# Sytronik/thesia

Measured on AMD Instinct MI355X. Metric: STFT frames/sec (whole step: STFT->dB->min/max->u16 image->level-0 RGBA raster), n_fft=2048, higher is better.
Workload: dtype f32

## Files before the change

__graft_entry__.py:

```python
from __future__ import annotations

import os
import shutil
import subprocess
import sys

ROOT = os.path.dirname(os.path.abspath(__file__))
CSRC = os.path.join(ROOT, "thesia_amd", "csrc")
LIB = os.path.join(ROOT, "thesia_amd", "libthesia_amd.so")
OBJDIR = os.path.join(ROOT, "build", "obj")
SOURCES = ["kernels_stft_w2048.hip", "kernels_stft_w4096.hip", "kernels_stft_w1024.hip", "kernels_stft.hip", "api.hip", "track_manager.hip", "track_manager_multi.hip", "kernels_stft_long.hip",
           "kernels_mel.hip", "kernels_image.hip", "kernels_waveform.hip", "kernels_loudness.hip", "kernels_dynamics.hip", "kernels_spectrum.hip", "kernels_meter.hip", "kernels_export.hip", "kernels_resample.hip", "host_math.cpp", "reader_plan.cpp", "batch_plan.cpp", "tile_cache.cpp"]
EXTRA_FLAGS = {"kernels_image.hip": ["-ffp-contract=off"], "kernels_waveform.hip": ["-ffp-contract=off"],
               "kernels_loudness.hip": ["-ffp-contract=off"],
               "kernels_dynamics.hip": ["-ffp-contract=off"],
               "kernels_spectrum.hip": ["-ffp-contract=off"],
               "kernels_meter.hip": ["-ffp-contract=off"],
               "kernels_export.hip": ["-ffp-contract=off"],
               "kernels_resample.hip": ["-ffp-contract=off", "-fno-slp-vectorize"],
               "kernels_stft.hip": ["-fno-slp-vectorize"] + os.environ.get("TH_STFT_EXTRA_FLAGS", "").split(),
               "kernels_stft_w1024.hip": ["-fno-slp-vectorize"] + os.environ.get("TH_STFT_EXTRA_FLAGS", "").split(),
               "kernels_stft_w2048.hip": ["-fno-slp-vectorize"] + os.environ.get("TH_STFT_EXTRA_FLAGS", "").split(),
               "kernels_stft_w4096.hip": ["-fno-slp-vectorize"] + os.environ.get("TH_STFT_EXTRA_FLAGS", "").split(),
               "kernels_stft_long.hip": ["-fno-slp-vectorize"]}
HEADERS = ["batch_plan.h", "common.h", "context.h", "export_core.h", "host_math.h", "kernels.h", "mel_fuse.h", "plan_error.h", "reader_plan.h", "resample_block.h", "resample_core.h", "stft_core.h", "stft_plan.h", "stft_pk.h", "stft_wave.h", "stft_wave_multi.h", "stft_block.h", "tile_cache.h", "track_manager_internal.h",
           "../../include/thesia_amd.h", "../../include/thesia_amd_testing.h"]


def _hipcc() -> str:
    for cand in (shutil.which("hipcc"), "/opt/rocm/bin/hipcc"):
        if cand and os.path.exists(cand):
            return cand
    raise RuntimeError("hipcc not found")


def _stale(target: str, deps) -> bool:
    if not os.path.exists(target):
        return True
    t = os.path.getmtime(target)
    return any(os.path.getmtime(d) > t for d in deps if os.path.exists(d))


def build(force: bool = False) -> None:
    import fcntl
    os.makedirs(OBJDIR, exist_ok=True)
    with open(os.path.join(OBJDIR, ".lock"), "w") as lock:
        fcntl.flock(lock, fcntl.LOCK_EX)
        try:
            _build_locked(force)
# ... 84 lines not shown
```

include/thesia_amd_testing.h:

```cpp
#ifndef THESIA_AMD_TESTING_H
#define THESIA_AMD_TESTING_H

#include "thesia_amd.h"

TH_API int th_plan_set_kernel(th_plan *plan, int which);

TH_API int th_build_ab_variants(void);

TH_API int th_plan_mel_moments_info(const th_plan *plan, uint32_t *n_groups, uint32_t *taps, double *max_dev, double *max_amp);

TH_API int th_plan_time_kernel(th_plan *plan, int enable);
TH_API int th_plan_kernel_ms_history(th_plan *plan, float *out_ms, size_t capacity, size_t *n_out);
TH_API int th_plan_last_kernel_ms(th_plan *plan, float *ms);

TH_API int th_tm_put_img(th_tm *tm, size_t id, uint32_t ch, const uint16_t *img, size_t height, size_t width);

#endif
```

thesia_amd/_ffi.py:

```python
from __future__ import annotations

import ctypes as C
import importlib.util
import os
import sys

_HERE = os.path.dirname(os.path.abspath(__file__))
LIB_PATH = os.environ.get("THESIA_AMD_LIB") or os.path.join(_HERE, "libthesia_amd.so")

if not os.path.exists(LIB_PATH):
    raise ImportError(
        f"{LIB_PATH} not found: build the HIP extension first "
        "(python -c 'import __graft_entry__ as g; g.build()').  thesia_amd has no CPU fallback."
    )



def _preload_hip_runtime() -> None:
    if "torch" in sys.modules or os.environ.get("THESIA_AMD_SYSTEM_HIP") == "1":
        return
    try:
        spec = importlib.util.find_spec("torch")
    except Exception:
        spec = None
# ... 207 lines not shown
    "th_host_alloc": [vp, C.c_size_t, C.POINTER(C.c_void_p)],
    "th_host_free": [vp, C.c_void_p],
    "th_minmax_reduce_dev": [vp, C.c_void_p, C.c_size_t, C.c_void_p],
    "th_global_db_range_dev": [vp, C.c_void_p, C.c_float, C.c_void_p],
    "th_minmax_reduce_range_dev": [vp, vp, C.c_size_t, C.c_float, vp, vp],
    "th_spec_to_img_batch_dev_ranged": [vp, C.POINTER(ImgDesc), C.c_size_t, C.c_void_p, C.c_uint32],
    "th_plan_time_kernel": [vp, C.c_int],
    "th_plan_last_kernel_ms": [vp, C.POINTER(C.c_float)],
    "th_plan_kernel_ms_history": [vp, c_f32p, C.c_size_t, c_szp],
    "th_channel_stats_dev": [vp, C.POINTER(StatsDesc), C.c_size_t, c_f32p, c_f32p],
    "th_audio_stats_dev": [vp, C.POINTER(AudioDesc), C.c_size_t, C.POINTER(AudioStats)],
    "th_k_weighting": [C.c_uint32, C.POINTER(C.c_double), C.POINTER(C.c_double)],
    "th_loudness_n_blocks": [C.c_size_t, C.c_uint32, c_szp],
    "th_gated_loudness": [C.POINTER(C.c_double), C.c_size_t, C.POINTER(C.c_double)],
    "th_tm_get_audio_stats": [vp, C.c_size_t, C.POINTER(AudioStats)],
    "th_tmg_get_audio_stats": [vp, C.c_size_t, C.POINTER(AudioStats)],
    "th_waveform_pyramid_bins": [C.c_uint64, C.c_uint32],
    "th_waveform_pyramid_offset": [C.c_uint64, C.c_uint32],
    "th_waveform_pyramid_dev": [vp, C.POINTER(PyramidDesc), C.c_size_t],
    "th_tm_tile_cache": [vp, C.POINTER(vp)],
    "th_tm_set_lod_source": [vp, C.c_int],
    "th_tm_mip_level": [vp, C.c_size_t, C.c_uint32, C.c_uint32, C.c_uint32, c_u16p, C.c_size_t, c_szp, c_szp],
    "th_tm_put_img": [vp, C.c_size_t, C.c_uint32, c_u16p, C.c_size_t, C.c_size_t],
    "th_tm_lod_footprint": [vp, c_szp, c_szp, c_szp],
    "th_tm_get_audio_render_metadata": [vp, C.c_size_t, C.c_uint32, C.c_double, C.c_int, C.POINTER(RenderMetadata)],
    "th_tmg_create": [C.POINTER(C.c_int), C.c_size_t, C.POINTER(vp)],
    "th_tmg_destroy": [vp],
    "th_tmg_n_devices": [vp, c_szp],
    "th_tmg_track_device": [vp, C.c_size_t, C.POINTER(C.c_uint32)],
    "th_tmg_set_colormap": [vp, c_u8p, C.c_size_t],
    "th_tmg_set_setting": [vp, C.c_double, C.c_uint32, C.c_uint32, C.c_int],
    "th_tmg_set_dB_range": [vp, C.c_float],
    "th_tmg_add_tracks": [vp, C.c_size_t, c_szp, C.POINTER(C.c_uint32), C.POINTER(C.c_uint32), C.POINTER(c_f32p),
                          c_szp],
    "th_tmg_remove_track": [vp, C.c_size_t],
    "th_tmg_apply_track_list_changes": [vp, c_szp, C.c_size_t, c_szp, C.POINTER(C.c_uint32)],
    "th_tmg_get_db_state": [vp, c_f32p, c_f32p, C.POINTER(C.c_uint32)],
    "th_tmg_spec_shape": [vp, C.c_size_t, C.c_uint32, c_szp, c_szp],
    "th_tmg_img_shape": [vp, C.c_size_t, C.c_uint32, c_szp, c_szp],
    "th_tmg_copy_spec": [vp, C.c_size_t, C.c_uint32, c_f32p, C.c_size_t],
    "th_tmg_copy_img": [vp, C.c_size_t, C.c_uint32, c_u16p, C.c_size_t],
    "th_tmg_revisions": [vp, C.POINTER(C.c_uint64), C.POINTER(C.c_uint64)],
    "th_tmg_get_spectrogram_tile": [vp, C.c_size_t, C.c_uint32, C.c_uint32, C.c_uint32, C.c_uint32, C.c_uint32,
                                    c_u8p, C.c_size_t, c_szp],
    "th_tmg_get_spectrogram_tiles": [vp, C.c_void_p, C.c_size_t, C.c_void_p, C.c_size_t, c_szp, c_szp],
    "th_tmg_get_waveform_tile": [vp, C.c_size_t, C.c_uint32, C.c_uint32, C.c_uint32, c_u8p, C.c_size_t, c_szp],
# ... 77 lines not shown
```

thesia_amd/csrc/api.hip:

```cpp
#include <hip/hip_runtime.h>

#include <cmath>
#include <cstdio>
#include <cstring>
#include <memory>
#include <mutex>
#include <vector>

#include "common.h"
#include "context.h"
#include "export_core.h"
#include "host_math.h"
#include "kernels.h"
#include "mel_fuse.h"
#include "resample_core.h"
#include "track_manager_internal.h"
#if !defined(TH_MEL_BAND_TAPS_2048)
#define TH_MEL_BAND_TAPS_2048 64u
#define TH_MEL_BAND_TAPS_1024 80u
#endif
#if !defined(TH_MEL_BAND_SPREAD)
#define TH_MEL_BAND_SPREAD 1
#endif

// ... 334 lines not shown
}
TH_API int th_timer_start(th_ctx *c) {
    TH_TRY
    TH_REQUIRE(c, "ctx is NULL");
    TH_HIP(hipSetDevice(c->device));
    TH_HIP(hipEventRecord(c->ev0, c->stream));
    return TH_OK;
    TH_CATCH
}
TH_API int th_timer_stop_ms(th_ctx *c, float *ms) {
    TH_TRY
    TH_CHECK(refuse_while_capturing("reading a timer"));
    TH_REQUIRE(c && ms, "NULL argument");
    TH_HIP(hipSetDevice(c->device));
    TH_HIP(hipEventRecord(c->ev1, c->stream));
    TH_HIP(hipEventSynchronize(c->ev1));
    TH_HIP(hipEventElapsedTime(ms, c->ev0, c->ev1));
    return TH_OK;
    TH_CATCH
}

namespace th {

int DeviceTable::ensure(size_t bytes) {
    if (bytes <= cap) return TH_OK;
    TH_CHECK(refuse_while_capturing("allocating a scratch buffer or a descriptor table"));
    if (dptr) {
        TH_HIP(hipFree(dptr));
        dptr = nullptr;
        cap = 0;
    }
    size_t want = bytes < 4096 ? 4096 : bytes + bytes / 2;
    TH_HIP(hipMalloc(&dptr, want));
    cap = want;
    last.clear();
    return TH_OK;
}

int DeviceTable::upload(hipStream_t s, const void *src, size_t bytes) {
    if (bytes == last.size() && bytes && std::memcmp(last.data(), src, bytes) == 0) return TH_OK;
    TH_CHECK(refuse_while_capturing("uploading a descriptor table (a first call, or one with other descriptors)"));
    TH_HIP(hipStreamSynchronize(s));
    int rc = ensure(bytes);
    if (rc != TH_OK) return rc;
    if (bytes) TH_HIP(hipMemcpy(dptr, src, bytes, hipMemcpyHostToDevice));
    last.assign(static_cast<const unsigned char *>(src), static_cast<const unsigned char *>(src) + bytes);
    return TH_OK;
}

void DeviceTable::release() {
    if (dptr) (void)hipFree(dptr);
    dptr = nullptr;
    cap = 0;
    last.clear();
}

}

static void resolve_route(th_plan &p) {
    using R = StftRoute;
    const StftGeom &g = p.g;
    const int k = p.kernel_choice, wv = p.wave_waves;
    R r;
    r.block_plan = stft_is_block_plan(g);
    const bool wave = k != SEL_GENERIC && stft_wave_supported(g) && (g.n_mel == 0 || p.d_mel_bt != nullptr);
    r.no_wave_kernel = k >= SEL_WAVE && !wave;
    r.long_plan = k == SEL_BLOCK ? 1 : k == SEL_SUBWAVE ? 2
                : (g.n_mel != 0 && g.log2_nc == 13 && p.d_mel_mom != nullptr && k != SEL_MEL_TWO_KERNELS) ? 1
                : stft_subwave_default(g) ? 2 : 1;
    bool fused = false, mom_small = false, bsum_fits = false;
    if (g.n_mel != 0 && wave && k != SEL_MEL_AMP && k != SEL_MEL_MFMA) {
        bsum_fits = k != SEL_MEL_PIECES && p.d_mel_bsum != nullptr && stft_wave_mel_fits(g, wv, p.mel_bsum_words, true);
        const bool pieces_fit = p.d_mel_fuse != nullptr && stft_wave_mel_fits(g, wv, p.mel_fuse_words);
        if (g.log2_nc >= 8 && g.log2_nc <= 10 && p.d_mel_mom != nullptr && k != SEL_MEL_TWO_KERNELS && k != SEL_MEL_PIECES)
            mom_small = g.log2_nc == 8 ? p.d_mel_rows == nullptr && stft_wave_multi_applies(g, 2) && stft_wave_multi_mel_fits(g, wv, 0)
                                       : !bsum_fits && !pieces_fit && stft_wave_mel_fits(g, wv, 0, true);
        if (g.log2_nc == 11)
            fused = k != SEL_MEL_TWO_KERNELS && p.d_mel_mom != nullptr && stft_wave_mel_fits(g, wv, 1, true);
        else if (g.log2_nc == 12 || g.log2_nc == 13)
// ... 30 lines not shown
    static const char *const main_name[] = {"stft_generic_kernel", "stft_bluestein_kernel", "stft_wave_kernel", "stft_wave_kernel",
                                            "stft_block_kernel", "stft_subwave_kernel"};
    static const char *const second_name[] = {"", "+mel_rows_kernel", "+mel_band_rows_kernel", "+mel_mfma_kernel"};
    std::snprintf(r.name, sizeof r.name, "%s%s%s", main_name[(int)r.main], fused ? "(fused mel)" : "", second_name[(int)r.mel_second]);
    p.route = r;
}

TH_API int th_plan_create(th_ctx *c, uint32_t sr, size_t win, size_t hop, size_t n_fft, int freq_scale,
                          size_t n_mel, th_plan **out) {
    TH_TRY
    TH_CHECK(refuse_while_capturing("creating a plan"));
    TH_REQUIRE(c && out, "NULL argument");
    *out = nullptr;
    TH_REQUIRE(freq_scale == TH_FREQ_LINEAR || freq_scale == TH_FREQ_MEL, "bad freq_scale %d", freq_scale);
    TH_REQUIRE(win > 1 && hop >= 1 && win <= n_fft, "need 1 < win <= n_fft and hop >= 1 (win=%zu hop=%zu n_fft=%zu)",
               win, hop, n_fft);
    TH_REQUIRE(sr > 0, "sr must be > 0");
    size_t odd_part = n_fft;
    while (odd_part > 1 && odd_part % 2 == 0) odd_part /= 2;
    if (n_fft < 2 || n_fft % 2 != 0 || n_fft > TH_MAX_N_FFT)
        return fail(TH_ERR_UNSUPPORTED, "n_fft=%zu: supported is every even n_fft from 2 to %u", n_fft, (unsigned)TH_MAX_N_FFT);
    TH_HIP(hipSetDevice(c->device));

    std::unique_ptr<th_plan> owner(new th_plan());
    th_plan *p = owner.get();
    p->ctx = c;
    p->sr = sr;
    p->freq_scale = freq_scale;
    StftGeom &g = p->g;
    g = stft_geom(win, hop, n_fft);

    const std::vector<float> w = normalized_hann(win, n_fft);
    const std::vector<cf32> tw = build_twiddles(n_fft);
    {
        const WaveWindowHost ww = build_wave_window(w.data(), win, n_fft, th::stft_wave_phased_mode(g, 0));
        TH_CHECK(p->d_wtab.fill(ww.wtab));
        if (!ww.phased.empty()) TH_CHECK(p->d_wtab_phased.fill(ww.phased));
    }
    TH_CHECK(p->d_window.fill(w));
    {
        const uint32_t zero[4] = {0, 0, 0, 0};
        TH_CHECK(p->d_queue_head.fill(zero, sizeof zero));
    }
    TH_CHECK(p->d_tw.fill(tw));
    if (odd_part > th::STFT_MAX_DIRECT_ODD) {
        const BluesteinTables bt = bluestein_tables(n_fft, th::stft_bluestein_m(g));
        TH_CHECK(p->d_bs_chirp.fill(bt.chirp));
// ... 1039 lines not shown
        dm = static_cast<unsigned char *>(c->loud_mem.dptr);
    }
    b->d_sums = reinterpret_cast<double *>(dm + o_sums);
    double *d_blk = reinterpret_cast<double *>(dm + o_blk), *d_z = reinterpret_cast<double *>(dm + o_z), *d_q = reinterpret_cast<double *>(dm + o_q);
    uint32_t *d_pk = reinterpret_cast<uint32_t *>(dm + o_sums + b->n_ch * 8);
    size_t si = 0;
    for (size_t t = 0, jc = 0; t < n; t++) {
        const size_t q0 = si;
        for (uint32_t k = 0; k < descs[t].n_channels; k++, jc++) {
            LoudJob &j = jobs[jc];
            j.z = d_z + 8 * si;
            j.q = d_q + si;
            j.sumsq = b->d_sums + jc;
            j.peak = d_pk + jc;
            si += j.n_fchunks;
        }
        tjobs[t].q = d_q + q0;
        tjobs[t].out = d_blk + b->blk0[t];
    }
    std::vector<unsigned char> h(o_sums, 0);
    std::memcpy(h.data(), jobs.data(), jobs.size() * sizeof(LoudJob));
    for (size_t r = 0; r < rates.size(); r++) std::memcpy(h.data() + o_rates + r * sizeof(LoudnessRate), rates[r], sizeof(LoudnessRate));
    std::memcpy(h.data() + o_tj, tjobs.data(), tjobs.size() * sizeof(LoudTrackJob));
    TH_HIP(hipMemcpy(dm, h.data(), o_sums, hipMemcpyHostToDevice));
    TH_HIP(hipMemsetAsync(b->d_sums, 0, sums_bytes, c->stream));
    TH_HIP(launch_loudness(reinterpret_cast<const LoudJob *>(dm), (uint32_t)jobs.size(), max_chunks, max_fchunks,
                           reinterpret_cast<const LoudnessRate *>(dm + o_rates), lds_floats, reinterpret_cast<const LoudTrackJob *>(dm + o_tj),
                           (uint32_t)n, max_blocks, c->stream));
    for (size_t t = 0; t < n; t++)
        if (descs[t].block_energy && tjobs[t].n_blocks)
            TH_HIP(hipMemcpyAsync(descs[t].block_energy, tjobs[t].out, tjobs[t].n_blocks * 8, hipMemcpyDeviceToDevice, c->stream));
    return TH_OK;
}

int loudness_collect(LoudnessBatch *b, bool sync_stream) {
    th_ctx *c = b->ctx;
    TH_HIP(hipSetDevice(c->device));
    const size_t sums_bytes = b->n_ch * 8 + (b->n_ch * 4 + 7) / 8 * 8;
    b->h_sums.assign(sums_bytes / 8 + b->n_blocks, 0.0);
    if (sync_stream) {
        TH_HIP(hipMemcpyAsync(b->h_sums.data(), b->d_sums, sums_bytes + b->n_blocks * 8, hipMemcpyDeviceToHost, c->stream));
        TH_HIP(hipStreamSynchronize(c->stream));
    } else {
        TH_HIP(hipMemcpy(b->h_sums.data(), b->d_sums, sums_bytes + b->n_blocks * 8, hipMemcpyDeviceToHost));
    }
    return TH_OK;
}
// ... 39 lines not shown
```

thesia_amd/csrc/context.h:

```cpp
#pragma once
#include <hip/hip_runtime.h>

#include <cstring>
#include <initializer_list>
#include <mutex>
#include <vector>

#include "common.h"
#include "stft_core.h"
#include "stft_plan.h"

namespace th {

template <class T>
struct DeviceBuf {
    T *ptr = nullptr;
    DeviceBuf() = default;
    DeviceBuf(const DeviceBuf &) = delete;
    DeviceBuf &operator=(const DeviceBuf &) = delete;
    DeviceBuf(DeviceBuf &&o) noexcept : ptr(o.ptr) { o.ptr = nullptr; }
    DeviceBuf &operator=(DeviceBuf &&o) noexcept {
        if (this != &o) {
            reset();
            ptr = o.ptr;
            o.ptr = nullptr;
        }
        return *this;
    }
    ~DeviceBuf() { reset(); }
    void reset() {
        if (ptr) (void)hipFree(ptr);
        ptr = nullptr;
    }
    T *get() const { return ptr; }
    operator T *() const { return ptr; }
    hipError_t alloc(size_t bytes) {
        reset();
        return hipMalloc((void **)&ptr, bytes);
    }
    int fill(const void *h, size_t bytes) {
        reset();
        void **d = (void **)&ptr;
        TH_HIP(hipMalloc(d, bytes));
        TH_HIP(hipMemcpy(*d, h, bytes, hipMemcpyHostToDevice));
        return TH_OK;
    }
    template <class V>
    int fill(const std::vector<V> &h) { return fill(h.data(), h.size() * sizeof(V)); }
};

struct DeviceTable {
    void *dptr = nullptr;
    size_t cap = 0;
    std::vector<unsigned char> last;
    int ensure(size_t bytes);
    int upload(hipStream_t s, const void *src, size_t bytes);
    void release();
    DeviceTable() = default;
    DeviceTable(const DeviceTable &) = delete;
    DeviceTable &operator=(const DeviceTable &) = delete;
    ~DeviceTable() { release(); }
};

struct KeyedTables {
    struct Src {
        const void *data;
        size_t bytes;
    };
    DeviceTable tab[3];
    std::vector<unsigned char> key;
    uint32_t n_blocks = 0;
    bool hit(const void *k, size_t bytes) const { return !key.empty() && key.size() == bytes && std::memcmp(key.data(), k, bytes) == 0; }
    int store(hipStream_t s, const void *k, size_t bytes, uint32_t blocks, std::initializer_list<Src> srcs) {
        key.clear();
        size_t i = 0;
        for (const Src &src : srcs) {
            if (src.bytes) TH_CHECK(tab[i].upload(s, src.data, src.bytes));
            i++;
        }
        key.assign(static_cast<const unsigned char *>(k), static_cast<const unsigned char *>(k) + bytes);
        n_blocks = blocks;
        return TH_OK;
    }
    template <class T>
    const T *at(size_t i) const { return static_cast<const T *>(tab[i].dptr); }
};

int refuse_while_capturing(const char *what);

}

struct th_ctx {
    int device = 0;
    uint32_t n_cu = 256;
    hipStream_t stream = nullptr;
    bool own_stream = false;
    hipStream_t capture_stream = nullptr;
    bool capture_swapped = false;
    hipEvent_t ev0 = nullptr, ev1 = nullptr;
    std::recursive_mutex mu;
    th::DeviceTable wave_jobs, wave_start, colormap, tile_out, lod_tabs, lod_tmp, pyr_jobs, pyr_sums, loud_mem;
    th::KeyedTables img, raster, fused;
    ~th_ctx() {
        if (ev0) (void)hipEventDestroy(ev0);
        if (ev1) (void)hipEventDestroy(ev1);
        if (own_stream && stream) (void)hipStreamDestroy(stream);
        if (capture_stream) (void)hipStreamDestroy(capture_stream);
    }
};

struct th_plan {
    th_ctx *ctx = nullptr;
    uint32_t sr = 0;
    int freq_scale = 0;
    int kernel_choice = 0;
    int wave_waves = 0;
    int wave_chunk = 0;
    static constexpr size_t TIMER_SLOTS = 64;
    bool time_kernel = false;
    uint64_t timed_launches = 0;
    std::vector<hipEvent_t> ev_k0, ev_k1;
    th::StftGeom g{};
    th::DeviceBuf<float> d_window;
    th::DeviceBuf<th::cf32> d_tw;
    th::DeviceBuf<double> d_bs_chirp, d_bs_bhat, d_bs_twm, d_bs_tws;
// ... 7 lines not shown
    std::vector<float> h_mel_fb;
    th::DeviceBuf<float> d_mel_bt;
    th::DeviceBuf<uint32_t> d_mel_band, d_mel_slice;
    uint32_t mel_kblocks = 0, mel_ntiles = 0, mel_zero_block = 0, mel_slices = 0;
    th::DeviceBuf<uint32_t> d_mel_rows;
    uint32_t mel_rows_groups = 0;
    th::DeviceTable amp_buf, mel_jobs, mel_tile_start;
    size_t amp_zeroed = 0;
    th::DeviceTable chunk_mm;
    th::DeviceTable gen_scratch;
    th::DeviceTable post_jobs;
    th::DeviceBuf<uint32_t> d_mel_fuse;
    uint32_t mel_fuse_words = 0, mel_fuse_slots = 0, mel_fuse_groups = 0;
    th::DeviceBuf<uint32_t> d_mel_bsum;
    uint32_t mel_bsum_words = 0, mel_bsum_groups = 0, mel_bsum_hdr[16] = {};
    th::DeviceBuf<th::cf32> d_twc;
    uint32_t mel_bsum_reach = 0;
    th::DeviceBuf<uint32_t> d_mel_mom;
    uint32_t mel_mom_groups = 0, mel_mom_taps = 0;
    double mel_mom_max_dev = 0.0, mel_mom_max_amp = 0.0;
    th::DeviceTable jobs, tile_start;
    th::DeviceTable edge_jobs, edge_tile_start;
    th::StftRoute route;
    ~th_plan() {
        for (hipEvent_t e : ev_k0) (void)hipEventDestroy(e);
        for (hipEvent_t e : ev_k1) (void)hipEventDestroy(e);
    }
};

namespace th {
struct LoudnessBatch {
    th_ctx *ctx = nullptr;
    DeviceBuf<unsigned char> d_own;
    double *d_sums = nullptr;
    size_t n_ch = 0, n_blocks = 0;
    std::vector<size_t> ch0, blk0;
    std::vector<uint32_t> srs;
    std::vector<uint64_t> ns;
    std::vector<double> h_blocks;
    std::vector<double> h_sums;
    LoudnessBatch() = default;
    LoudnessBatch(const LoudnessBatch &) = delete;
    LoudnessBatch &operator=(const LoudnessBatch &) = delete;
    ~LoudnessBatch();
};
int loudness_enqueue(th_ctx *c, const th_audio_desc *descs, size_t n, bool own_memory, bool allow_bad_rate, LoudnessBatch *b);
// ... 4 lines not shown
```

thesia_amd/csrc/track_manager.hip:

```cpp
#include <hip/hip_runtime.h>

#include <cmath>
#include <condition_variable>
#include <cstring>
#include <chrono>
#include <list>
#include <map>
#include <memory>
#include <set>
#include <thread>
#include <atomic>
#include <shared_mutex>
#include <tuple>
#include <vector>

#include "common.h"
#include "context.h"
#include "export_core.h"
#include "host_math.h"
#include "kernels.h"
#include "resample_core.h"
#include "tile_cache.h"
#include "track_manager_internal.h"

// ... 79 lines not shown
    uint32_t max_sr = 0;
    float dB_range = 100.f;
    uint32_t colormap_length = 258;
    std::vector<size_t> no_spec_img_ids;
    std::map<size_t, Track> tracks;
    std::map<PlanKey, th_plan *> plans;
    std::vector<uint8_t> colormap_rgba{0, 0, 0, 255, 255, 255, 255, 255};
    DeviceBuf<uint8_t> d_colormap;
    th_tile_cache cache{th_tile_cache::DEFAULT_BUDGET};
    mutable std::shared_mutex rw;
    std::mutex slot_mu;
    std::condition_variable slot_cv;
    std::vector<std::unique_ptr<ReaderSlot>> slots;
    int lod_source = 0;
    int norm_kind = TH_NORM_OFF;
    float norm_target = 0.0f;
    int guard_mode = TH_GUARD_REDUCE_GLOBAL_LEVEL;
    std::map<std::pair<uint32_t, uint32_t>, AxisTable> axis_tabs;
    th::DeviceTable mip_jobs;
    th::DeviceTable mip_scratch;
    std::list<std::vector<unsigned char>> axis_staging;
    hipStream_t copy_stream = nullptr;
    hipEvent_t copy_ev = nullptr;
    hipEvent_t img_ev = nullptr, mips_ev = nullptr;
    bool img_ev_recorded = false;
    uint64_t stat_tiles_served = 0;
    std::mutex batch_mu;
    void *batch_stage = nullptr, *batch_stage_dev = nullptr;
    size_t batch_stage_cap = 0;

    void invalidate_waveform() { cache.invalidate_waveform(); }
    void invalidate_spectrogram() { cache.invalidate_spectrogram(); }
    void invalidate_all() { cache.invalidate_all(); }
    uint64_t waveform_revision() const {
        std::lock_guard<std::mutex> lk(cache.mu);
        return cache.waveform_revision;
    }
    uint64_t spectrogram_revision() const {
        std::lock_guard<std::mutex> lk(cache.mu);
        return cache.spectrogram_revision;
    }
};

namespace {

void free_mips(Channel &c) {
// ... 553 lines not shown
int writer_done(th_tm *tm, int rc) {
    hipError_t e = hipStreamSynchronize(tm->ctx->stream);
    tm->axis_staging.clear();
    tm->img_ev_recorded = false;
    if (rc == TH_OK && e != hipSuccess) TH_HIP(e);
    return rc;
}

int writer_done_images(th_tm *tm, int rc) {
    if (rc != TH_OK || !tm->img_ev_recorded || tm->lod_source != 0) return writer_done(tm, rc);
    const hipError_t e = hipEventSynchronize(tm->img_ev);
    tm->img_ev_recorded = false;
    if (e != hipSuccess) TH_HIP(e);
    return TH_OK;
}

}

TH_API int th_tm_create(th_ctx *c, th_tm **out) {
    TH_TRY
    TH_REQUIRE(c && out, "NULL argument");
    std::unique_ptr<th_tm> tm(new th_tm());
    tm->ctx = c;
    TH_HIP(hipSetDevice(c->device));
    hipError_t e = hipStreamCreateWithFlags(&tm->copy_stream, hipStreamNonBlocking);
    if (e == hipSuccess) e = hipEventCreateWithFlags(&tm->copy_ev, hipEventDisableTiming);
    if (e == hipSuccess) e = hipEventCreateWithFlags(&tm->img_ev, hipEventDisableTiming);
    if (e == hipSuccess) e = hipEventCreateWithFlags(&tm->mips_ev, hipEventDisableTiming);
    if (e != hipSuccess) {
        if (tm->mips_ev) (void)hipEventDestroy(tm->mips_ev);
        if (tm->img_ev) (void)hipEventDestroy(tm->img_ev);
        if (tm->copy_ev) (void)hipEventDestroy(tm->copy_ev);
        if (tm->copy_stream) (void)hipStreamDestroy(tm->copy_stream);
        TH_HIP(e);
    }
    *out = tm.release();
    return TH_OK;
    TH_CATCH
}

TH_API int th_tm_destroy(th_tm *tm) {
    TH_TRY
    if (!tm) return TH_OK;
    (void)hipSetDevice(tm->ctx->device);
    (void)hipStreamSynchronize(tm->ctx->stream);
    for (auto &sp : tm->slots) {
// ... 1 lines not shown
        (void)hipStreamDestroy(sp->stream);
        (void)hipHostFree(sp->h_tile);
        if (sp->exp_copy) (void)hipStreamDestroy(sp->exp_copy);
        for (int b = 0; b < 2; b++) {
            if (sp->exp_done[b]) (void)hipEventDestroy(sp->exp_done[b]);
            if (sp->exp_copied[b]) (void)hipEventDestroy(sp->exp_copied[b]);
        }
    }
    tm->tracks.clear();
    for (auto &kv : tm->plans) th_plan_destroy(kv.second);
    tm->axis_tabs.clear();
    if (tm->batch_stage) (void)hipHostFree(tm->batch_stage);
    tm->mip_jobs.release();
    tm->mip_scratch.release();
    tm->d_colormap.reset();
    if (tm->copy_ev) (void)hipEventDestroy(tm->copy_ev);
    if (tm->img_ev) (void)hipEventDestroy(tm->img_ev);
    if (tm->mips_ev) (void)hipEventDestroy(tm->mips_ev);
    if (tm->copy_stream) {
        (void)hipStreamSynchronize(tm->copy_stream);
        (void)hipStreamDestroy(tm->copy_stream);
    }
    delete tm;
    return TH_OK;
    TH_CATCH
}

namespace {
int upload_colormap(th_tm *tm) {
    if (tm->d_colormap) TH_CHECK(free_checked(tm->d_colormap));
    TH_HIP(tm->d_colormap.alloc(tm->colormap_rgba.size()));
    TH_HIP(hipMemcpyAsync(tm->d_colormap, tm->colormap_rgba.data(), tm->colormap_rgba.size(), hipMemcpyHostToDevice,
                          tm->ctx->stream));
    TH_HIP(hipStreamSynchronize(tm->ctx->stream));
    return TH_OK;
}
}

TH_API int th_tm_set_colormap(th_tm *tm, const uint8_t *rgba, size_t bytes) {
    TH_TRY
    TH_REQUIRE(tm && rgba, "NULL argument");
    std::unique_lock<std::shared_mutex> wl(tm->rw);
    int rc = tmi::set_colormap_only(tm, rgba, bytes);
    if (rc != TH_OK) return rc;
    tm->invalidate_spectrogram();
    std::vector<size_t> upd;
// ... 1120 lines not shown
    th_tm *tm = stg.tm;
    TH_CHECK(derive_enqueue(tm, trs, stg.derive.get()));
    std::vector<SpecInput> chans;
    for (auto &it : trs) {
        const Track &tr = *it.second;
        const Derived &d = stg.derive->of[it.first];
        if (!d.active && !tr.d_dyn && tr.ch[0].has_spec) continue;
        for (size_t k = 0; k < tr.ch.size(); k++)
            chans.push_back({it.first, (uint32_t)k, tr.sr, d.active ? d.aud[k] : tr.ch[k].d_orig, tr.ch[k].n});
    }
    TH_CHECK(compute_specs(tm, setting_of(tm), chans, stg.created, &stg.fresh));
    TH_HIP(hipStreamSynchronize(tm->ctx->stream));
    return derive_collect(trs, stg.derive.get());
}

struct AddArgs {
    size_t n_tracks;
    const size_t *ids;
    const uint32_t *srs, *n_channels;
    const float *const *channels_flat;
    const size_t *n_samples;
    std::map<size_t, size_t> last_of;
    std::vector<size_t> flat0;
};
struct AddInFlight {
    std::vector<PendingMinMax> pending;
    std::vector<std::unique_ptr<LoudnessBatch>> loud;
    std::vector<std::pair<size_t, size_t>> loud_ids;
};

constexpr size_t GROUP_BYTES = (size_t)96 << 20;

int stage_group(Staged &stg, const AddArgs &a, size_t *t, AddInFlight *fl, double *t_launch) {
    th_tm *tm = stg.tm;
    th_ctx *c = tm->ctx;
    std::vector<SpecInput> chans;
    std::vector<th_pyramid_desc> pdescs;
    std::vector<th_audio_desc> adescs;
    std::vector<std::vector<const float *>> aptrs;
    for (size_t bytes = 0; *t < a.n_tracks && (bytes == 0 || bytes < GROUP_BYTES); ++*t) {
        const size_t i = *t, id = a.ids[i], n = a.n_samples[i];
        if (a.last_of.at(id) != i) continue;
        Track &tr = stg.tracks[id];
        tr.sr = a.srs[i];
        tr.ch.resize(a.n_channels[i]);
        tr.guard_stats.assign(tr.ch.size(), th_guard_clip_stats{});
        const PoolLayout pl = pool_layout(n, 1);
        TH_HIP(tr.d_pool.alloc(pl.stride * tr.ch.size() * sizeof(float)));
        aptrs.emplace_back();
        for (uint32_t k = 0; k < a.n_channels[i]; k++) {
            Channel &ch = tr.ch[k];
            ch.n = n;
            ch.pyr_levels = pl.levels;
            ch.d_wav = ch.d_draw = ch.d_orig = tr.d_pool.get() + (size_t)k * pl.stride;
            ch.d_pyr = ch.d_pyr_orig = ch.d_wav + pl.wav_f;
            TH_HIP(hipMemcpyAsync(ch.d_wav, a.channels_flat[a.flat0[i] + k], n * sizeof(float), hipMemcpyHostToDevice, tm->copy_stream));
            bytes += n * sizeof(float);
            chans.push_back({id, k, tr.sr, ch.d_wav, n});
            pdescs.push_back(th_pyramid_desc{ch.d_wav, ch.d_pyr, n, ch.pyr_levels, PYR_FIRST});
            aptrs.back().push_back(ch.d_wav);
        }
        adescs.push_back(th_audio_desc{nullptr, (uint64_t)n, a.n_channels[i], a.srs[i], nullptr});
        fl->loud_ids.emplace_back(id, fl->loud.size());
// ... 67 lines not shown
    std::vector<std::pair<size_t, Track *>> trs;
    for (auto &kv : tm->tracks) trs.push_back({kv.first, &kv.second});
    TH_CHECK(stage_derived(*stg, trs));
    *out = std::move(stg);
    return TH_OK;
}

void get_common_dynamics(th_tm *tm, int *kind, float *target, int *mode) {
    if (kind) *kind = tm->norm_kind;
    if (target) *target = tm->norm_target;
    if (mode) *mode = tm->guard_mode;
}

int prepare_add(th_tm *tm, size_t n_tracks, const size_t *ids, const uint32_t *srs, const uint32_t *n_channels,
                const float *const *channels_flat, const size_t *n_samples, StagedPtr *out) {
    th_ctx *c = tm->ctx;
    TH_HIP(hipSetDevice(c->device));
    TH_REQUIRE(tm->copy_stream != nullptr && tm->copy_ev != nullptr, "manager without its copy stream");
    AddInFlight fl;
    StagedPtr stg(new Staged(tm));
    const bool prof = getenv("TH_TM_PROF") != nullptr;
    auto now = []() { return std::chrono::duration<double, std::milli>(std::chrono::steady_clock::now().time_since_epoch()).count(); };
    const double tp0 = now();
    AddArgs a{n_tracks, ids, srs, n_channels, channels_flat, n_samples, {}, std::vector<size_t>(n_tracks, 0)};
    for (size_t t = 0, flat = 0; t < n_tracks; t++) {
        a.last_of[ids[t]] = t;
        a.flat0[t] = flat;
        flat += n_channels[t];
        stg->added.insert(ids[t]);
    }
    double t_launch = 0.0;
    for (size_t t = 0; t < n_tracks;) TH_CHECK(stage_group(*stg, a, &t, &fl, &t_launch));
    const double tp1 = now();
    TH_HIP(hipStreamSynchronize(tm->copy_stream));
    TH_HIP(hipStreamSynchronize(c->stream));
    int rc = collect_added(*stg, &fl);
    if (rc == TH_OK && tm->norm_kind != TH_NORM_OFF) {
        stg->derive.reset(new DeriveBatch);
        get_common_dynamics(tm, &stg->derive->kind, &stg->derive->target, &stg->derive->mode);
        std::vector<std::pair<size_t, Track *>> trs;
        for (auto &kv : stg->tracks) trs.push_back({kv.first, &kv.second});
        rc = stage_derived(*stg, trs);
    }
    if (prof) fprintf(stderr, "th_tm_add_tracks prof: staging + launches %.2f ms (of which pyramid / STFT launches %.2f), drain %.2f\n", tp1 - tp0, t_launch, now() - tp1);
    if (rc != TH_OK) return rc;
    *out = std::move(stg);
    return TH_OK;
}

void commit(th_tm *tm, StagedPtr s) {
    (void)hipSetDevice(tm->ctx->device);
    for (auto &kv : s->tracks) tm->tracks[kv.first] = std::move(kv.second);
    if (s->derive) {
// ... 420 lines not shown
```

Measured before the change: 293.6 million.

## Stage descriptor table uploads through pinned ring buffers and size add-track groups adaptively

Descriptor table uploads no longer synchronize the stream and do a blocking hipMemcpy. They now copy through a ring of pinned host slots with events, and grown device buffers are retired and recycled instead of freed synchronously. Track-add staging groups are sized from the remaining bytes, with a minimum that depends on whether the host audio is pinned. The aim is to remove host-device stalls per upload, in exchange for more bookkeeping, a mutex, and pinned host memory.

```diff
diff --git a/__graft_entry__.py b/__graft_entry__.py
--- a/__graft_entry__.py
+++ b/__graft_entry__.py
@@ -23,8 +23,8 @@
                "kernels_stft_w2048.hip": ["-fno-slp-vectorize"] + os.environ.get("TH_STFT_EXTRA_FLAGS", "").split(),
                "kernels_stft_w4096.hip": ["-fno-slp-vectorize"] + os.environ.get("TH_STFT_EXTRA_FLAGS", "").split(),
                "kernels_stft_long.hip": ["-fno-slp-vectorize"]}
-HEADERS = ["batch_plan.h", "common.h", "context.h", "export_core.h", "host_math.h", "kernels.h", "mel_fuse.h", "plan_error.h", "reader_plan.h", "resample_block.h", "resample_core.h", "stft_core.h", "stft_plan.h", "stft_pk.h", "stft_wave.h", "stft_wave_multi.h", "stft_block.h", "tile_cache.h", "track_manager_internal.h",
-           "../../include/thesia_amd.h", "../../include/thesia_amd_testing.h"]
+HEADERS = ["batch_plan.h", "common.h", "context.h", "export_core.h", "host_math.h", "kernels.h", "mel_fuse.h", "plan_error.h", "reader_plan.h", "resample_block.h", "resample_core.h", "stft_core.h", "stft_plan.h", "stft_pk.h", "stft_wave.h", "stft_wave_multi.h", "stft_block.h", "table_staging.h", "tile_cache.h", "track_manager_internal.h",
+           "../../include/thesia_amd.h", "../../include/thesia_amd_testing.h", "../../include/thesia_amd_testing_hooks.h"]
 
 
 def _hipcc() -> str:
diff --git a/include/thesia_amd_testing.h b/include/thesia_amd_testing.h
--- a/include/thesia_amd_testing.h
+++ b/include/thesia_amd_testing.h
@@ -15,4 +15,6 @@
 
 TH_API int th_tm_put_img(th_tm *tm, size_t id, uint32_t ch, const uint16_t *img, size_t height, size_t width);
 
+#include "thesia_amd_testing_hooks.h"
+
 #endif
diff --git a/include/thesia_amd_testing_hooks.h b/include/thesia_amd_testing_hooks.h
--- /dev/null
+++ b/include/thesia_amd_testing_hooks.h
@@ -0,0 +1,12 @@
+#ifndef THESIA_AMD_TESTING_HOOKS_H
+#define THESIA_AMD_TESTING_HOOKS_H
+
+#include "thesia_amd.h"
+
+TH_API int th_testing_set_table_staging(uint32_t slots, size_t slot_bytes);
+
+TH_API int th_testing_table_uploads(uint64_t *uploads, uint64_t *host_waits);
+
+TH_API int th_tm_set_add_group_bytes(th_tm *tm, size_t bytes);
+
+#endif
diff --git a/thesia_amd/_ffi.py b/thesia_amd/_ffi.py
--- a/thesia_amd/_ffi.py
+++ b/thesia_amd/_ffi.py
@@ -253,6 +253,9 @@
     "th_tm_set_lod_source": [vp, C.c_int],
     "th_tm_mip_level": [vp, C.c_size_t, C.c_uint32, C.c_uint32, C.c_uint32, c_u16p, C.c_size_t, c_szp, c_szp],
     "th_tm_put_img": [vp, C.c_size_t, C.c_uint32, c_u16p, C.c_size_t, C.c_size_t],
+    "th_testing_set_table_staging": [C.c_uint32, C.c_size_t],
+    "th_testing_table_uploads": [C.POINTER(C.c_uint64), C.POINTER(C.c_uint64)],
+    "th_tm_set_add_group_bytes": [vp, C.c_size_t],
     "th_tm_lod_footprint": [vp, c_szp, c_szp, c_szp],
     "th_tm_get_audio_render_metadata": [vp, C.c_size_t, C.c_uint32, C.c_double, C.c_int, C.POINTER(RenderMetadata)],
     "th_tmg_create": [C.POINTER(C.c_int), C.c_size_t, C.POINTER(vp)],
diff --git a/thesia_amd/csrc/api.hip b/thesia_amd/csrc/api.hip
--- a/thesia_amd/csrc/api.hip
+++ b/thesia_amd/csrc/api.hip
@@ -1,5 +1,6 @@
 #include <hip/hip_runtime.h>
 
+#include <atomic>
 #include <cmath>
 #include <cstdio>
 #include <cstring>
@@ -380,6 +381,105 @@
 
 namespace th {
 
+namespace {
+std::atomic<uint64_t> g_staging_gen{0};
+std::atomic<uint32_t> g_staging_slots{0};
+std::atomic<size_t> g_staging_slot_bytes{0};
+std::atomic<uint64_t> g_table_uploads{0}, g_staging_waits{0};
+
+struct HipStaging final : StagingDevice {
+    hipStream_t s;
+    hipError_t err = hipSuccess;
+    explicit HipStaging(hipStream_t stream) : s(stream) {}
+    bool ok(hipError_t e) {
+        if (e != hipSuccess && err == hipSuccess) err = e;
+        return e == hipSuccess;
+    }
+    bool issue(void **ev) override {
+        hipEvent_t e = static_cast<hipEvent_t>(*ev);
+        if (!e && !ok(hipEventCreateWithFlags(&e, hipEventDisableTiming))) return false;
+        *ev = e;
+        return ok(hipEventRecord(e, s));
+    }
+    bool query(void *ev, bool *done) override {
+        const hipError_t e = hipEventQuery(static_cast<hipEvent_t>(ev));
+        *done = e == hipSuccess;
+        if (e == hipErrorNotReady) (void)hipGetLastError();
+        return e == hipSuccess || e == hipErrorNotReady;
+    }
+    bool wait(void *ev) override {
+        g_staging_waits++;
+        return ok(hipEventSynchronize(static_cast<hipEvent_t>(ev)));
+    }
+    void drop(void *ev) override { (void)hipEventDestroy(static_cast<hipEvent_t>(ev)); }
+    void *host_alloc(size_t bytes) override {
+        void *p = nullptr;
+        return ok(hipHostMalloc(&p, bytes, hipHostMallocDefault)) ? p : nullptr;
+    }
+    void host_free(void *p) override { (void)hipHostFree(p); }
+    void device_free(void *p) override { (void)hipFree(p); }
+};
+}
+
+int StagedCopier::copy(hipStream_t s, void *dst, const void *src, size_t bytes) {
+    HipStaging dev(s);
+    std::lock_guard<std::mutex> lk(mu);
+    const uint64_t gen = g_staging_gen.load();
+    if (gen != geometry_gen) {
+        const uint32_t slots = g_staging_slots.load();
+        const bool ok = book.set_geometry(dev, slots ? StagingGeometry{slots, g_staging_slot_bytes.load()} : geometry);
+        geometry_gen = gen;
+        if (!ok) TH_HIP(dev.err != hipSuccess ? dev.err : hipErrorUnknown);
+    }
+    if (!book.reap(dev)) TH_HIP(dev.err != hipSuccess ? dev.err : hipErrorUnknown);
+    const unsigned char *from = static_cast<const unsigned char *>(src);
+    unsigned char *to = static_cast<unsigned char *>(dst);
+    for (size_t off = 0; off < bytes;) {
+        const size_t n = book.piece(bytes - off);
+        void *mem = nullptr;
+        if (!book.acquire(dev, n, &mem)) TH_HIP(dev.err != hipSuccess ? dev.err : hipErrorOutOfMemory);
+        std::memcpy(mem, from + off, n);
+        TH_HIP(hipMemcpyAsync(to + off, mem, n, hipMemcpyHostToDevice, s));
+        if (!book.submitted(dev)) {
+            (void)hipStreamSynchronize(s);
+            TH_HIP(dev.err != hipSuccess ? dev.err : hipErrorUnknown);
+        }
+        off += n;
+    }
+    return TH_OK;
+}
+
+int StagedCopier::retire(hipStream_t s, void *dptr, size_t bytes) {
+    HipStaging dev(s);
+    std::lock_guard<std::mutex> lk(mu);
+    if (book.retire(dev, dptr, bytes)) return TH_OK;
+    (void)hipStreamSynchronize(s);
+    TH_HIP(hipFree(dptr));
+    return TH_OK;
+}
+
+int StagedCopier::fresh_buffer(hipStream_t s, size_t want, void **dptr, size_t *cap) {
+    HipStaging dev(s);
+    {
+        std::lock_guard<std::mutex> lk(mu);
+        if (!book.reap(dev)) TH_HIP(dev.err != hipSuccess ? dev.err : hipErrorUnknown);
+        if (book.take(want, dptr, cap)) return TH_OK;
+    }
+    TH_HIP(hipMalloc(dptr, want));
+    *cap = want;
+    return TH_OK;
+}
+
+void StagedCopier::give(void *dptr, size_t bytes) {
+    std::lock_guard<std::mutex> lk(mu);
+    book.give(dptr, bytes);
+}
+
+void StagedCopier::release() {
+    HipStaging dev(nullptr);
+    book.release(dev);
+}
+
 int DeviceTable::ensure(size_t bytes) {
     if (bytes <= cap) return TH_OK;
     TH_CHECK(refuse_while_capturing("allocating a scratch buffer or a descriptor table"));
@@ -398,21 +498,53 @@
 int DeviceTable::upload(hipStream_t s, const void *src, size_t bytes) {
     if (bytes == last.size() && bytes && std::memcmp(last.data(), src, bytes) == 0) return TH_OK;
     TH_CHECK(refuse_while_capturing("uploading a descriptor table (a first call, or one with other descriptors)"));
-    TH_HIP(hipStreamSynchronize(s));
-    int rc = ensure(bytes);
-    if (rc != TH_OK) return rc;
-    if (bytes) TH_HIP(hipMemcpy(dptr, src, bytes, hipMemcpyHostToDevice));
+    last.clear();
+    StagedCopier &cp = shared ? *shared : up;
+    if (bytes > cap) {
+        void *fresh = nullptr, *old = dptr;
+        size_t got = 0;
+        const size_t had = cap;
+        TH_CHECK(cp.fresh_buffer(s, bytes < 4096 ? 4096 : bytes + bytes / 2, &fresh, &got));
+        dptr = fresh;
+        cap = got;
+        if (old) TH_CHECK(cp.retire(s, old, had));
+    }
+    if (bytes) {
+        TH_CHECK(cp.copy(s, dptr, src, bytes));
+        g_table_uploads++;
+    }
     last.assign(static_cast<const unsigned char *>(src), static_cast<const unsigned char *>(src) + bytes);
     return TH_OK;
 }
 
 void DeviceTable::release() {
-    if (dptr) (void)hipFree(dptr);
+    up.release();
+    if (dptr && shared) shared->give(dptr, cap);
+    else if (dptr) (void)hipFree(dptr);
     dptr = nullptr;
     cap = 0;
     last.clear();
 }
 
+}
+
+TH_API int th_testing_set_table_staging(uint32_t slots, size_t slot_bytes) {
+    TH_TRY
+    TH_REQUIRE((slots == 0) == (slot_bytes == 0), "slots and slot_bytes: both 0 (the default) or both positive");
+    TH_REQUIRE(slots <= 1024, "at most 1024 slots");
+    g_staging_slots = slots;
+    g_staging_slot_bytes = slot_bytes;
+    g_staging_gen++;
+    return TH_OK;
+    TH_CATCH
+}
+
+TH_API int th_testing_table_uploads(uint64_t *uploads, uint64_t *host_waits) {
+    TH_TRY
+    if (uploads) *uploads = g_table_uploads.load();
+    if (host_waits) *host_waits = g_staging_waits.load();
+    return TH_OK;
+    TH_CATCH
 }
 
 static void resolve_route(th_plan &p) {
@@ -489,7 +621,7 @@
         return fail(TH_ERR_UNSUPPORTED, "n_fft=%zu: supported is every even n_fft from 2 to %u", n_fft, (unsigned)TH_MAX_N_FFT);
     TH_HIP(hipSetDevice(c->device));
 
-    std::unique_ptr<th_plan> owner(new th_plan());
+    std::unique_ptr<th_plan> owner(new th_plan(c));
     th_plan *p = owner.get();
     p->ctx = c;
     p->sr = sr;
@@ -1575,7 +1707,7 @@
     std::memcpy(h.data(), jobs.data(), jobs.size() * sizeof(LoudJob));
     for (size_t r = 0; r < rates.size(); r++) std::memcpy(h.data() + o_rates + r * sizeof(LoudnessRate), rates[r], sizeof(LoudnessRate));
     std::memcpy(h.data() + o_tj, tjobs.data(), tjobs.size() * sizeof(LoudTrackJob));
-    TH_HIP(hipMemcpy(dm, h.data(), o_sums, hipMemcpyHostToDevice));
+    TH_CHECK(c->stage.copy(c->stream, dm, h.data(), o_sums));
     TH_HIP(hipMemsetAsync(b->d_sums, 0, sums_bytes, c->stream));
     TH_HIP(launch_loudness(reinterpret_cast<const LoudJob *>(dm), (uint32_t)jobs.size(), max_chunks, max_fchunks,
                            reinterpret_cast<const LoudnessRate *>(dm + o_rates), lds_floats, reinterpret_cast<const LoudTrackJob *>(dm + o_tj),
diff --git a/thesia_amd/csrc/context.h b/thesia_amd/csrc/context.h
--- a/thesia_amd/csrc/context.h
+++ b/thesia_amd/csrc/context.h
@@ -9,6 +9,7 @@
 #include "common.h"
 #include "stft_core.h"
 #include "stft_plan.h"
+#include "table_staging.h"
 
 namespace th {
 
@@ -49,10 +50,28 @@
     int fill(const std::vector<V> &h) { return fill(h.data(), h.size() * sizeof(V)); }
 };
 
+struct StagedCopier {
+    std::mutex mu;
+    TableStaging book;
+    StagingGeometry geometry;
+    uint64_t geometry_gen = 0;
+    int copy(hipStream_t s, void *dst, const void *src, size_t bytes);
+    int retire(hipStream_t s, void *dptr, size_t bytes);
+    int fresh_buffer(hipStream_t s, size_t want, void **dptr, size_t *cap);
+    void give(void *dptr, size_t bytes);
+    void release();
+    explicit StagedCopier(StagingGeometry g = STAGING_DEFAULT) : book(g), geometry(g) {}
+    StagedCopier(const StagedCopier &) = delete;
+    StagedCopier &operator=(const StagedCopier &) = delete;
+    ~StagedCopier() { release(); }
+};
+
 struct DeviceTable {
     void *dptr = nullptr;
     size_t cap = 0;
     std::vector<unsigned char> last;
+    StagedCopier up;
+    StagedCopier *shared = nullptr;
     int ensure(size_t bytes);
     int upload(hipStream_t s, const void *src, size_t bytes);
     void release();
@@ -99,8 +118,14 @@
     bool capture_swapped = false;
     hipEvent_t ev0 = nullptr, ev1 = nullptr;
     std::recursive_mutex mu;
+    th::StagedCopier stage{th::STAGING_SHARED};
     th::DeviceTable wave_jobs, wave_start, colormap, tile_out, lod_tabs, lod_tmp, pyr_jobs, pyr_sums, loud_mem;
     th::KeyedTables img, raster, fused;
+    th_ctx() {
+        for (th::DeviceTable *t : {&wave_jobs, &wave_start, &colormap, &lod_tabs, &pyr_jobs}) t->shared = &stage;
+        for (th::KeyedTables *k : {&img, &raster, &fused})
+            for (th::DeviceTable &t : k->tab) t.shared = &stage;
+    }
     ~th_ctx() {
         if (ev0) (void)hipEventDestroy(ev0);
         if (ev1) (void)hipEventDestroy(ev1);
@@ -154,6 +179,9 @@
     th::DeviceTable jobs, tile_start;
     th::DeviceTable edge_jobs, edge_tile_start;
     th::StftRoute route;
+    explicit th_plan(th_ctx *c) : ctx(c) {
+        for (th::DeviceTable *t : {&mel_jobs, &mel_tile_start, &post_jobs, &jobs, &tile_start, &edge_jobs, &edge_tile_start}) t->shared = &c->stage;
+    }
     ~th_plan() {
         for (hipEvent_t e : ev_k0) (void)hipEventDestroy(e);
         for (hipEvent_t e : ev_k1) (void)hipEventDestroy(e);
diff --git a/thesia_amd/csrc/table_staging.h b/thesia_amd/csrc/table_staging.h
--- /dev/null
+++ b/thesia_amd/csrc/table_staging.h
@@ -0,0 +1,155 @@
+#pragma once
+#include <cstddef>
+#include <cstdint>
+#include <deque>
+#include <initializer_list>
+#include <vector>
+
+namespace th {
+
+struct StagingDevice {
+    virtual ~StagingDevice() = default;
+    virtual bool issue(void **ev) = 0;
+    virtual bool query(void *ev, bool *done) = 0;
+    virtual bool wait(void *ev) = 0;
+    virtual void drop(void *ev) = 0;
+    virtual void *host_alloc(size_t bytes) = 0;
+    virtual void host_free(void *p) = 0;
+    virtual void device_free(void *p) = 0;
+};
+
+struct StagingGeometry {
+    uint32_t slots;
+    size_t slot_bytes;
+};
+constexpr StagingGeometry STAGING_DEFAULT{4, (size_t)64 << 10};
+constexpr StagingGeometry STAGING_SHARED{64, (size_t)64 << 10};
+
+class TableStaging {
+  public:
+    struct Slot {
+        void *mem = nullptr;
+        void *ev = nullptr;
+        bool pending = false;
+    };
+    struct Retired {
+        void *dptr;
+        size_t bytes;
+        void *ev;
+    };
+    static constexpr size_t SPARES_MAX = 32;
+    uint64_t host_waits = 0, host_allocs = 0, device_frees = 0;
+
+    explicit TableStaging(StagingGeometry g = STAGING_DEFAULT) : geo_(g) {}
+
+    const StagingGeometry &geometry() const { return geo_; }
+    size_t retired() const { return retired_.size(); }
+    size_t spares() const { return spare_.size(); }
+    size_t pending() const {
+        size_t n = 0;
+        for (const Slot &s : slots_) n += s.pending;
+        return n;
+    }
+    size_t piece(size_t left) const { return left < geo_.slot_bytes ? left : geo_.slot_bytes; }
+
+    bool acquire(StagingDevice &d, size_t bytes, void **mem) {
+        if (bytes > geo_.slot_bytes) return false;
+        if (slots_.empty()) slots_.resize(geo_.slots);
+        Slot &s = slots_[next_];
+        if (s.pending) {
+            bool done = false;
+            if (!d.query(s.ev, &done)) return false;
+            if (!done) {
+                host_waits++;
+                if (!d.wait(s.ev)) return false;
+            }
+            s.pending = false;
+        }
+        if (!arena_) {
+            arena_ = d.host_alloc(geo_.slot_bytes * slots_.size());
+            if (!arena_) return false;
+            host_allocs++;
+            for (size_t i = 0; i < slots_.size(); i++) slots_[i].mem = static_cast<unsigned char *>(arena_) + i * geo_.slot_bytes;
+        }
+        cur_ = next_;
+        next_ = (next_ + 1) % slots_.size();
+        *mem = s.mem;
+        return true;
+    }
+    bool submitted(StagingDevice &d) {
+        Slot &s = slots_[cur_];
+        if (!d.issue(&s.ev)) return false;
+        s.pending = true;
+        return true;
+    }
+
+    bool retire(StagingDevice &d, void *dptr, size_t bytes) {
+        void *ev = nullptr;
+        if (!d.issue(&ev)) return false;
+        retired_.push_back(Retired{dptr, bytes, ev});
+        return true;
+    }
+    bool reap(StagingDevice &d) {
+        while (!retired_.empty()) {
+            bool done = false;
+            if (!d.query(retired_.front().ev, &done)) return false;
+            if (!done) break;
+            d.drop(retired_.front().ev);
+            retired_.front().ev = nullptr;
+            spare_.push_back(retired_.front());
+            retired_.pop_front();
+        }
+        while (spare_.size() > SPARES_MAX) {
+            d.device_free(spare_.front().dptr);
+            spare_.pop_front();
+            device_frees++;
+        }
+        return true;
+    }
+    void give(void *dptr, size_t bytes) { spare_.push_back(Retired{dptr, bytes, nullptr}); }
+    bool take(size_t bytes, void **dptr, size_t *cap) {
+        size_t best = spare_.size();
+        for (size_t i = 0; i < spare_.size(); i++)
+            if (spare_[i].bytes >= bytes && (best == spare_.size() || spare_[i].bytes < spare_[best].bytes)) best = i;
+        if (best == spare_.size()) return false;
+        *dptr = spare_[best].dptr;
+        *cap = spare_[best].bytes;
+        spare_.erase(spare_.begin() + (long)best);
+        return true;
+    }
+
+    bool set_geometry(StagingDevice &d, StagingGeometry g) {
+        if (g.slots == 0 || g.slot_bytes == 0) return false;
+        bool ok = true;
+        for (Slot &s : slots_)
+            if (s.pending && !d.wait(s.ev)) ok = false;
+        drop_slots(d);
+        geo_ = g;
+        return ok;
+    }
+    void release(StagingDevice &d) {
+        drop_slots(d);
+        for (std::deque<Retired> *q : {&retired_, &spare_})
+            for (; !q->empty(); q->pop_front(), device_frees++) {
+                d.device_free(q->front().dptr);
+                if (q->front().ev) d.drop(q->front().ev);
+            }
+    }
+
+  private:
+    void drop_slots(StagingDevice &d) {
+        for (Slot &s : slots_)
+            if (s.ev) d.drop(s.ev);
+        if (arena_) d.host_free(arena_);
+        arena_ = nullptr;
+        slots_.clear();
+        next_ = cur_ = 0;
+    }
+    StagingGeometry geo_;
+    std::vector<Slot> slots_;
+    void *arena_ = nullptr;
+    size_t next_ = 0, cur_ = 0;
+    std::deque<Retired> retired_, spare_;
+};
+
+}
diff --git a/thesia_amd/csrc/track_manager.hip b/thesia_amd/csrc/track_manager.hip
--- a/thesia_amd/csrc/track_manager.hip
+++ b/thesia_amd/csrc/track_manager.hip
@@ -125,6 +125,7 @@
     std::list<std::vector<unsigned char>> axis_staging;
     hipStream_t copy_stream = nullptr;
     hipEvent_t copy_ev = nullptr;
+    size_t add_group_bytes = 0;
     hipEvent_t img_ev = nullptr, mips_ev = nullptr;
     bool img_ev_recorded = false;
     uint64_t stat_tiles_served = 0;
@@ -724,6 +725,7 @@
     TH_REQUIRE(c && out, "NULL argument");
     std::unique_ptr<th_tm> tm(new th_tm());
     tm->ctx = c;
+    tm->mip_jobs.shared = &c->stage;
     TH_HIP(hipSetDevice(c->device));
     hipError_t e = hipStreamCreateWithFlags(&tm->copy_stream, hipStreamNonBlocking);
     if (e == hipSuccess) e = hipEventCreateWithFlags(&tm->copy_ev, hipEventDisableTiming);
@@ -771,6 +773,15 @@
         (void)hipStreamDestroy(tm->copy_stream);
     }
     delete tm;
+    return TH_OK;
+    TH_CATCH
+}
+
+TH_API int th_tm_set_add_group_bytes(th_tm *tm, size_t bytes) {
+    TH_TRY
+    TH_REQUIRE(tm, "tm is NULL");
+    std::unique_lock<std::shared_mutex> wl(tm->rw);
+    tm->add_group_bytes = bytes;
     return TH_OK;
     TH_CATCH
 }
@@ -1937,6 +1948,9 @@
     const size_t *n_samples;
     std::map<size_t, size_t> last_of;
     std::vector<size_t> flat0;
+    std::vector<size_t> rest;
+    size_t fixed_group_bytes;
+    size_t group_min_bytes;
 };
 struct AddInFlight {
     std::vector<PendingMinMax> pending;
@@ -1944,7 +1958,18 @@
     std::vector<std::pair<size_t, size_t>> loud_ids;
 };
 
-constexpr size_t GROUP_BYTES = (size_t)96 << 20;
+constexpr size_t GROUP_MIN_BYTES_PINNED = (size_t)24 << 20, GROUP_MIN_BYTES_PAGEABLE = (size_t)192 << 20;
+constexpr size_t GROUP_SHARE_NUM = 4, GROUP_SHARE_DEN = 7;
+size_t group_target(const AddArgs &a, size_t rest) {
+    if (a.fixed_group_bytes) return a.fixed_group_bytes;
+    return std::max(a.group_min_bytes, rest / GROUP_SHARE_DEN * GROUP_SHARE_NUM);
+}
+bool is_pinned_host(const void *p) {
+    hipPointerAttribute_t at{};
+    const hipError_t e = hipPointerGetAttributes(&at, p);
+    if (e != hipSuccess) (void)hipGetLastError();
+    return e == hipSuccess && at.type == hipMemoryTypeHost;
+}
 
 int stage_group(Staged &stg, const AddArgs &a, size_t *t, AddInFlight *fl, double *t_launch) {
     th_tm *tm = stg.tm;
@@ -1953,7 +1978,8 @@
     std::vector<th_pyramid_desc> pdescs;
     std::vector<th_audio_desc> adescs;
     std::vector<std::vector<const float *>> aptrs;
-    for (size_t bytes = 0; *t < a.n_tracks && (bytes == 0 || bytes < GROUP_BYTES); ++*t) {
+    const size_t target = group_target(a, a.rest[*t]), join = a.fixed_group_bytes ? 0 : a.group_min_bytes / 2;
+    for (size_t bytes = 0; *t < a.n_tracks && (bytes < target || a.rest[*t] < join); ++*t) {
         const size_t i = *t, id = a.ids[i], n = a.n_samples[i];
         if (a.last_of.at(id) != i) continue;
         Track &tr = stg.tracks[id];
@@ -2067,13 +2093,19 @@
     const bool prof = getenv("TH_TM_PROF") != nullptr;
     auto now = []() { return std::chrono::duration<double, std::milli>(std::chrono::steady_clock::now().time_since_epoch()).count(); };
     const double tp0 = now();
-    AddArgs a{n_tracks, ids, srs, n_channels, channels_flat, n_samples, {}, std::vector<size_t>(n_tracks, 0)};
+    AddArgs a{n_tracks, ids, srs, n_channels, channels_flat, n_samples, {}, std::vector<size_t>(n_tracks, 0), std::vector<size_t>(n_tracks + 1, 0), tm->add_group_bytes, GROUP_MIN_BYTES_PAGEABLE};
     for (size_t t = 0, flat = 0; t < n_tracks; t++) {
         a.last_of[ids[t]] = t;
         a.flat0[t] = flat;
         flat += n_channels[t];
         stg->added.insert(ids[t]);
     }
+    for (size_t t = 0; t < n_tracks; t++)
+        if (a.last_of[ids[t]] == t && n_channels[t] && n_samples[t]) {
+            if (is_pinned_host(channels_flat[a.flat0[t]])) a.group_min_bytes = GROUP_MIN_BYTES_PINNED;
+            break;
+        }
+    for (size_t t = n_tracks; t-- > 0;) a.rest[t] = a.rest[t + 1] + (a.last_of[ids[t]] == t ? (size_t)n_channels[t] * n_samples[t] * sizeof(float) : 0);
     double t_launch = 0.0;
     for (size_t t = 0; t < n_tracks;) TH_CHECK(stage_group(*stg, a, &t, &fl, &t_launch));
     const double tp1 = now();
```

Result: no change. 293.4 million (median of 2 runs) (-0.1%).
